# mcahny/vps

Hardware: AMD Instinct MI355X
Metric: frames/sec FuseTrack 1024x2048 (higher is better)
Workload: dtype f32-grade: f16x3 split operands (fp16 pair with scaled residual, 22 significand bits) on MFMA, f32 accumulate

## Files before the change

### include/vps_hip.h

```cpp
#ifndef VPS_HIP_H
#define VPS_HIP_H

#include <stdint.h>

#ifdef __cplusplus
extern "C" {
#endif

int vps_abi_version(void);
const char* vps_build_info(void);

enum { VPS_ACT_NONE = 0, VPS_ACT_RELU = 1, VPS_ACT_LEAKY = 2 };
enum { VPS_PREC_F32 = 0, VPS_PREC_BF16 = 1, VPS_PREC_BF16X3 = 2, VPS_PREC_BF16X6 = 3, VPS_PREC_F16X3 = 4 };

typedef struct vps_conv_desc {
    const float* in;
    int32_t N, H, W;
    int32_t in_ld;
    int32_t in_coff;
    int32_t cin_pad;
    const float* w;
    int32_t cout, cout_pad, kpad;
    int32_t KH, KW, stride;
    int32_t pad_y[2], pad_x[2];
// ... 13 lines not shown
    int32_t off_ld;
    int32_t tile_n;
    int32_t ksplit;
    float* ws;
    int32_t prec;
    const void* w_split;
    int32_t korder;
    int32_t* status;
    double* gn_stats;
    int32_t gn_cpg, gn_rep;
    int32_t* tile_counter;
    const void* w_thin;
} vps_conv_desc;

int vps_conv2d(const vps_conv_desc* d, void* stream);

typedef struct vps_tensor4 {
    float* p;
    int64_t sn, sc, sh, sw;
} vps_tensor4;

int vps_resample2d(vps_tensor4 in, vps_tensor4 flow, vps_tensor4 out,
                   int B, int C, int H, int W, void* stream);

int vps_channelnorm(vps_tensor4 in, vps_tensor4 out, int B, int C, int H, int W, void* stream);

int vps_correlation(const float* in1, int ld1, int coff1, const float* in2, int ld2, int coff2,
                    float* out, int out_ld, int out_coff,
                    int N, int H, int W, int C, int max_disp, int stride2,
                    int act, float slope, void* stream);
// ... 1 lines not shown
                        float* out, int out_ld, int out_coff, int N, int H, int W, int C,
                        int max_disp, int stride2, int act, float slope, int32_t* status, void* stream);

int vps_flow_warp(const float* in, int in_ld, int in_coff, const float* flow, int flow_ld, int flow_coff,
                  float* out, int out_ld, int out_coff, int N, int H, int W, int C, void* stream);

int vps_nchw_to_nhwc(const float* in, float* out, int out_ld, int out_coff, int N, int C, int H, int W,
                     int Cpad, void* stream);
int vps_nhwc_to_nchw(const float* in, int in_ld, int in_coff, float* out, int N, int C, int H, int W, void* stream);

int vps_resize(const float* in, int in_ld, int in_coff, int Hi, int Wi,
               float* out, int out_ld, int out_coff, int Ho, int Wo,
               int N, int C, int mode, float alpha, void* stream);
int vps_pool3x3s2(const float* in, int in_ld, int in_coff, int Hi, int Wi,
                  float* out, int out_ld, int out_coff, int N, int C, int mode, void* stream);
int vps_bfp_gather(const float* const* levels, const int* ld, const int* ratio, int nlevels,
                   float* out, int out_ld, int out_coff, int N, int H0, int W0, int C, void* stream);
int vps_bfp_scatter(const float* bsf, int bsf_ld, const float* level, int lvl_ld, float* out, int out_ld,
                    int N, int H0, int W0, int C, int ratio, void* stream);
int vps_bfp_scatter_all(const float* bsf, int bsf_ld, const float* const* levels, const int* lvl_ld, float* const* outs,
                        const int* out_ld, int nlevels, int N, int H0, int W0, int C, void* stream);
int vps_axpb(const float* in, int in_ld, int in_coff, float* out, int out_ld, int out_coff,
             int64_t npix, int C, float a, float b, void* stream);

int vps_flow_prep(const float* img, const float* ref, const float* mean3, const float* std3,
                  float* out, int out_ld, int H, int W, double* partial, int nblk, float* rgb_mean_out,
                  void* stream);
int vps_flow_prep_pad(const float* img, const float* ref, const float* mean3, const float* std3,
                      float* out, int out_ld, int H, int W, int Hp, int Wp, double* partial, int nblk, float* rgb_mean_out,
                      void* stream);
// ... 4 lines not shown

int vps_flow_stage_full(const float* x6, int x_ld, const float* flow_a, int a_ld, int a_coff,
                        const float* flow_b, int b_ld, int b_coff, int H, int W, int mode, float mul,
                        float* out, int out_ld, void* stream);

int vps_groupnorm_relu(const float* in, int in_ld, float* out, int out_ld, int out_coff, int64_t npix, int C, int G,
                       const float* gamma, const float* beta, float eps, int relu,
                       double* stats, void* stream);
int vps_groupnorm_apply(const float* in, int in_ld, float* out, int out_ld, int out_coff, int64_t npix, int C, int G,
                        const float* gamma, const float* beta, float eps, int relu,
                        const double* stats, int nrep, void* stream);

int vps_tcea_temporal(const float* emb, int emb_ld, const float* emb_ref, int ref_ld,
                      const float* fea0, int f0_ld, const float* fea1, int f1_ld,
                      float* out, int out_ld, int64_t npix, int C, void* stream);
int vps_tcea_modulate(const float* fea, const float* att, const float* att_add, float* out,
                      int64_t n, void* stream);
int vps_tcea_modulate_ld(const float* fea, int fea_ld, const float* att, int att_ld, const float* att_add, int add_ld,
                         float* out, int out_ld, int64_t npix, int C, void* stream);

int vps_roi_align(const float* const* feats, const int* ld, const int* Hs, const int* Ws, const float* scales,
                  int nlevels, float finest_scale, const float* rois, int R, int C, int P, int sample_num,
                  float* out, void* stream);

int vps_nms_batched(const float* boxes, int nbatch, int nmax, const int32_t* counts_dev, float thr,
                    uint64_t* mask_ws, int32_t* keep, int32_t* nkeep, void* stream);

int vps_delta2bbox(const float* anchors, const float* deltas, const float* scores, float* boxes5, int n,
                   float std_x, float std_y, float std_w, float std_h, float img_h, float img_w, void* stream);

// ... 125 lines not shown
```

### vps_amd/csrc/conv_mfma.hip

```cpp
#include "conv_common.h"

namespace {
template <int TM, int TN, int WAVES_M, int WAVES_N, bool DEFORM>
__global__ __launch_bounds__(256, 2)
void conv_mfma_f32_kernel(const vps_conv_desc d, const int M, const int tiles_m, const int tiles_n,
                          const int ksteps_per_split) {
    constexpr int BN = WAVES_N * TN * 32;
    static_assert(WAVES_M * TM * 32 == BM, "block M tile must be 128");
    static_assert(WAVES_M * WAVES_N == 4, "4 wavefronts per block");
    constexpr int NB = BN / 32;

    __shared__ __attribute__((aligned(16))) float As[BM * LDS_LD];
    __shared__ __attribute__((aligned(16))) float Bs[BN * LDS_LD];

    const int t = threadIdx.x;
    int swz = xcd_swizzle(blockIdx.x, gridDim.x);
    int tile_n, tile_m, cls, split;
    decode_tile(d, swz, tiles_n, tiles_m, tile_n, tile_m, cls, split);

    const int py = cls / d.os_x, px = cls - py * d.os_x;
    const int pad_y = d.pad_y[py], pad_x = d.pad_x[px];
    const float* __restrict__ wcls = d.w + (size_t)cls * d.cout_pad * d.kpad;

    const int H = d.H, W = d.W, KH = d.KH, KW = d.KW, cin_pad = d.cin_pad;
// ... 777 lines not shown
        case CONV_K_H8: vpsi_launch_conv_h8(d, p, s); break;
        case CONV_K_PW: vpsi_launch_conv_pw(d, p, s); break;
        case CONV_K_Q: vpsi_launch_conv_q(d, p, s); break;
        default:
            if (d.tile_n == 128) launch_conv<2, 2, 2, 2>(d, p, s);
            else if (d.tile_n == 64) launch_conv<2, 1, 2, 2>(d, p, s);
            else launch_conv<1, 1, 4, 1>(d, p, s);
    }
    int st = vps_launch_status();
    if (st || !p.needs_reduce) return st;
    const size_t total = (size_t)d.nclass * p.M * d.cout;
    if (p.reduce_v4) hipLaunchKernelGGL(conv_splitk_reduce_kernel<4>, dim3(stream_grid((long)(total / 4), 256)), dim3(256), 0, s, d, p.M);
    else hipLaunchKernelGGL(conv_splitk_reduce_kernel<1>, dim3(stream_grid((long)total, 256)), dim3(256), 0, s, d, p.M);
    return vps_launch_status();
}
```

### vps_amd/csrc/conv_plan.h

```cpp
#pragma once
#include <stddef.h>
#include "../../include/vps_hip.h"

#ifndef VPS_EARG
#define VPS_EARG(x) (-1000 - (x))
#endif

enum conv_kernel {
    CONV_K_NONE = 0,
    CONV_K_SMALL3X3V,
    CONV_K_SMALL_BATCHED,
    CONV_K_SMALL,
    CONV_K_THIN,
    CONV_K_DCN256,
    CONV_K_N16T,
    CONV_K_N32,
    CONV_K_N16,
    CONV_K_H8S2,
    CONV_K_H8P,
    CONV_K_H8,
    CONV_K_HALO,
    CONV_K_PW,
    CONV_K_Q,
    CONV_K_F32,
// ... 29 lines not shown
    bool h8p;
    bool n16t;
    bool n32;
    bool s2_halo;
    bool thin;
    bool debug_occ;
};

struct conv_thin_shape { int c4, ks, s, ph; };
extern const conv_thin_shape conv_thin_shapes[4];

int vpsi_conv_check(const vps_conv_desc& d);
conv_plan vpsi_conv_plan(const vps_conv_desc& d, const conv_limits& lim, const conv_switches& sw);
const char* vpsi_conv_kernel_name(int kernel);

#ifdef __HIPCC__
void vpsi_launch_conv_small(const vps_conv_desc& d, const conv_plan& p, hipStream_t s);
void vpsi_launch_conv_thin(const vps_conv_desc& d, const conv_plan& p, hipStream_t s);
void vpsi_launch_conv_n16(const vps_conv_desc& d, const conv_plan& p, hipStream_t s);
void vpsi_launch_conv_h8(const vps_conv_desc& d, const conv_plan& p, hipStream_t s);
void vpsi_launch_conv_h8p(const vps_conv_desc& d, const conv_plan& p, hipStream_t s);
void vpsi_launch_conv_h8s2(const vps_conv_desc& d, const conv_plan& p, hipStream_t s);
void vpsi_launch_conv_pw(const vps_conv_desc& d, const conv_plan& p, hipStream_t s);
void vpsi_launch_conv_q(const vps_conv_desc& d, const conv_plan& p, hipStream_t s);
void vpsi_conv_pw_limits(conv_limits& lim, bool debug);
void vpsi_conv_thin_limits(conv_limits& lim, bool debug);
void vpsi_conv_q_debug_occ();
#endif
```

### vps_amd/csrc/conv_pw.hip

```cpp
#include "conv_common.h"
#include <cstdio>

namespace {

constexpr int PMODE = VPS_PREC_F16X3;

template <int TN, bool HAS_RES, int NKU>
__global__ __launch_bounds__(256, 2)
void conv_pw_kernel(const vps_conv_desc d, const int M, const int tiles_m, const int tiles_n, const int nk, const int nit) {
    constexpr int TM = 2, WAVES_N = 2;
    constexpr int BN = WAVES_N * TN * 32;
    typedef Split<PMODE> SM;
    typedef _Float16 elem_t;
    typedef vec8<elem_t> x8;
    typedef vec4<elem_t> x4;
    constexpr int NSA = SM::NSA, NSB = SM::NSB, NLB = SM::NLB, NT = SM::NT;
    static_assert(NSA == 2 && NLB == 2 && NSB == 3 && NT == 3, "f16x3");
    constexpr int ABUF = NSA * BM * LDS_LDH;
    constexpr int NFRAG = NLB * 2 * (BN / 32);
    constexpr int BBUF = NFRAG * 512;
    static_assert((NFRAG * 64) % 256 == 0, "whole 16-byte chunks per thread");
    constexpr int NBL = NFRAG * 64 / 256;
    constexpr int NST = TM * TN * 4;

// ... 12 lines not shown

    const int k4 = t & 7;
    const int r0 = t >> 3;
    const int nbt = d.cout_pad >> 5, kst = d.kpad >> 4;
    const size_t wplane = (size_t)nbt * kst * 512;
    const __amdgpu_buffer_rsrc_t wrsrc = make_rsrc(d.w_split, (unsigned)(wplane * NSB * sizeof(elem_t)));
    const unsigned wbase = (unsigned)((((size_t)(tile_n * (BN / 32)) * kst) * 512) * sizeof(elem_t));
    const unsigned wlane = (unsigned)lane * 16u;
    const __amdgpu_buffer_rsrc_t arsrc = make_rsrc(d.in, (unsigned)((size_t)d.N * d.H * d.W * d.in_ld * sizeof(float)));
    const __amdgpu_buffer_rsrc_t orsrc = make_rsrc(d.out, (unsigned)((size_t)d.N * d.Ho * d.Wo * d.out_ld * sizeof(float)));
    const int rs = d.res_shift;
    const __amdgpu_buffer_rsrc_t rrsrc = make_rsrc(HAS_RES ? d.res : d.in, HAS_RES ? (unsigned)((size_t)d.N * (d.Ho >> rs) * (d.Wo >> rs) * d.res_ld * sizeof(float)) : 0u);
    const unsigned ld4 = (unsigned)d.in_ld * 4u;
    const unsigned acoff = (unsigned)(d.in_coff + k4 * 4) * 4u;
    const bool plain = d.stride == 1;

    int lk = 0, lit = 0, bk = 0;
    unsigned rowoff[4];
    auto set_rows = [&](const int it) {
        const int tm = (it * mper + mlocal) * 8 + xcd;
#pragma unroll
        for (int i = 0; i < 4; ++i) {
            const int m = tm * BM + r0 + 32 * i;
            const bool ok = tm < tiles_m && m < M;
            unsigned pix = (unsigned)m;
            if (!plain) {
                const int mm = ok ? m : 0;
                const int qx = mm % d.Qw, tq = mm / d.Qw;
                const int qy = tq % d.Qh, n = tq / d.Qh;
                pix = (unsigned)((n * d.H + qy * d.stride) * d.W + qx * d.stride);
            }
            rowoff[i] = ok ? pix * ld4 + acoff : 0xFFFFFFF0u;
        }
    };
    f32x4 areg[2][4];
    x8 breg[2][NBL];
    float amax = 0.f;

    auto load_A = [&](const int slot) {
        const unsigned koff = (unsigned)lk * (BK * 4u);
#pragma unroll
        for (int i = 0; i < 4; ++i)
            areg[slot][i] = buffer_load16<f32x4>(arsrc, rowoff[i] != 0xFFFFFFF0u ? rowoff[i] + koff : 0xFFFFFFF0u, 0u);
        if (++lk == nk) {
            lk = 0;
            ++lit;
            set_rows(lit);
        }
    };
    auto load_B = [&](const int slot) {
#pragma unroll
        for (int j = 0; j < NBL; ++j) {
            const int f = wave + 4 * j, bcol = f % (BN / 32), pm = f / (BN / 32);
            breg[slot][j] = buffer_load16<x8>(wrsrc, wlane, wbase + (unsigned)(((size_t)(pm >> 1) * wplane + ((size_t)bcol * kst + 2 * bk + (pm & 1)) * 512) * sizeof(elem_t)));
        }
        if (++bk == nk) bk = 0;
    };
    auto store_A = [&](const int i, const int buf, const int slot) {
        x4 sp[NSA];
        split_act<PMODE>(areg[slot][i], sp, amax);
        const int row = r0 + 32 * i;
#pragma unroll
        for (int p = 0; p < NSA; ++p)
            *reinterpret_cast<x4*>(&As[buf * ABUF + p * (BM * LDS_LDH) + row * LDS_LDH + (((k4 >> 1) ^ lds_swz(row)) << 3) + ((k4 & 1) << 2)]) = sp[p];
    };
    auto store_B = [&](const int j, const int buf, const int slot) {
        *reinterpret_cast<x8*>(&Bs[buf * BBUF + (t + 256 * j) * 8]) = breg[slot][j];
    };

    const int frag_row = (wm * TM * 32 + (lane & 31)) * LDS_LDH;
    const int frag_sw = lds_swz(lane & 31);
    const int frag_chunk[2] = {(((lane >> 5)) ^ frag_sw) << 3, ((2 + (lane >> 5)) ^ frag_sw) << 3};
    x8 af[2][NSA][TM];
    x8 bf[NSB][TN];
    auto read_A = [&](const int m, const int buf) {
// ... 222 lines not shown
                for (int a = 0; a < TM; ++a)
#pragma unroll
                    for (int b = 0; b < TN; ++b)
#pragma unroll
                        for (int r = 0; r < 16; ++r) acc[a][b][r] = 0.f;
            }
        }
    }
    report_range<PMODE>(d, amax);
}

}

__attribute__((visibility("hidden")))
void vpsi_conv_pw_limits(conv_limits& lim, bool debug) {
    (void)hipOccupancyMaxActiveBlocksPerMultiprocessor(&lim.pw_per_cu[0], conv_pw_kernel<1, false, 0>, 256, 0);
    (void)hipOccupancyMaxActiveBlocksPerMultiprocessor(&lim.pw_per_cu[1], conv_pw_kernel<2, false, 0>, 256, 0);
    if (debug) for (int tn = 1; tn <= 2; ++tn) fprintf(stderr, "[vps] pointwise kernel <TN %d>: %d blocks/CU\n", tn, lim.pw_per_cu[tn - 1]);
}

__attribute__((visibility("hidden")))
void vpsi_launch_conv_pw(const vps_conv_desc& d, const conv_plan& p, hipStream_t s) {
    const int tn = d.tile_n == 128 ? 2 : 1;
#define VPS_PW_LAUNCH(TNV, RESV, NKV) hipLaunchKernelGGL((conv_pw_kernel<TNV, RESV, NKV>), dim3(p.grid), dim3(p.block), 0, s, d, p.M, p.tiles_m, p.tiles_n, p.nk, p.nit)
#define VPS_PW_NK(TNV, RESV)                                         \
    do {                                                             \
        if (p.nk == 2) VPS_PW_LAUNCH(TNV, RESV, 2);                  \
        else if (p.nk == 4) VPS_PW_LAUNCH(TNV, RESV, 4);             \
        else if (p.nk == 8) VPS_PW_LAUNCH(TNV, RESV, 8);             \
        else VPS_PW_LAUNCH(TNV, RESV, 0);                            \
    } while (0)
    if (d.res) { if (tn == 2) VPS_PW_NK(2, true); else VPS_PW_NK(1, true); }
    else { if (tn == 2) VPS_PW_NK(2, false); else VPS_PW_NK(1, false); }
#undef VPS_PW_NK
#undef VPS_PW_LAUNCH
}
```

### vps_amd/csrc/nn_ops.hip

```cpp
#include "common.h"

typedef float f32x4 __attribute__((ext_vector_type(4)));

namespace {

template <int V> struct vecn { typedef float type; };
template <> struct vecn<4> { typedef f32x4 type; };

template <int V>
__global__ __launch_bounds__(256)
void resize_kernel(const float* __restrict__ in, int in_ld, int in_coff, int Hi, int Wi,
                   float* __restrict__ out, int out_ld, int out_coff, int Ho, int Wo,
                   int N, int C, int mode, float alpha, float sh, float sw) {
    typedef typename vecn<V>::type vt;
    const int cv = C / V;
    const long total = (long)N * Ho * Wo * cv;
    for (long idx = (long)blockIdx.x * blockDim.x + threadIdx.x; idx < total; idx += (long)gridDim.x * blockDim.x) {
        const int c = (int)(idx % cv) * V;
        const int pix = (int)(idx / cv);
        const int x = pix % Wo;
        const int yy = pix / Wo;
        const int y = yy % Ho, n = yy / Ho;
        const float* ib = in + (size_t)n * Hi * Wi * in_ld + in_coff + c;
        vt v;
// ... 43 lines not shown
        }
        vt m = t[4], s = vt{}, zero = vt{};
#pragma unroll
        for (int k = 0; k < 9; ++k) {
            if constexpr (V == 1) { m = fmaxf(m, t[k]); }
            else {
#pragma unroll
                for (int e = 0; e < 4; ++e) m[e] = fmaxf(m[e], t[k][e]);
            }
            s += ok[k] ? t[k] : zero;
        }
        *reinterpret_cast<vt*>(out + (size_t)pix * out_ld + out_coff + c) = mode == 0 ? m : s / 9.0f;
    }
}

struct GatherArgs {
    const float* lv[5];
    int ld[5];
    int ratio[5];
    int n;
};

__global__ __launch_bounds__(256)
void bfp_gather_kernel(GatherArgs a, float* __restrict__ out, int out_ld, int out_coff, int N, int H0, int W0, int C) {
    const int c4n = C >> 2;
    const long total = (long)N * H0 * W0 * c4n;
    const float div = (float)a.n;
    for (long idx = (long)blockIdx.x * blockDim.x + threadIdx.x; idx < total; idx += (long)gridDim.x * blockDim.x) {
        const int c4 = (int)(idx % c4n);
        const long pix = idx / c4n;
// ... 256 lines not shown
            cor0 += __shfl_xor(cor0, off, 64);
            cor1 += __shfl_xor(cor1, off, 64);
        }
        const float p0 = 1.f / (1.f + expf(-cor0));
        const float p1 = 1.f / (1.f + expf(-cor1));
        for (int c4 = lane; c4 < c4n; c4 += 64) {
            const f32x4 f0 = *reinterpret_cast<const f32x4*>(fea0 + (size_t)pix * f0_ld + 4 * c4);
            const f32x4 f1 = *reinterpret_cast<const f32x4*>(fea1 + (size_t)pix * f1_ld + 4 * c4);
            *reinterpret_cast<f32x4*>(out + (size_t)pix * out_ld + 4 * c4) = f0 * p0;
            *reinterpret_cast<f32x4*>(out + (size_t)pix * out_ld + C + 4 * c4) = f1 * p1;
        }
    }
}

__global__ __launch_bounds__(256)
void tcea_modulate_kernel(const float* __restrict__ fea, const float* __restrict__ att, const float* __restrict__ att_add,
                          float* __restrict__ out, long n) {
    for (long i = (long)blockIdx.x * blockDim.x + threadIdx.x; i < n; i += (long)gridDim.x * blockDim.x) {
        const float s = 1.f / (1.f + expf(-att[i]));
        out[i] = fea[i] * s * 2.f + att_add[i];
    }
}

__global__ __launch_bounds__(256)
void tcea_modulate_ld_kernel(const float* __restrict__ fea, int fea_ld, const float* __restrict__ att, int att_ld,
                             const float* __restrict__ att_add, int add_ld, float* __restrict__ out, int out_ld, long npix, int C) {
    const int c4n = C >> 2;
    const long total = npix * c4n;
    for (long i = (long)blockIdx.x * blockDim.x + threadIdx.x; i < total; i += (long)gridDim.x * blockDim.x) {
        const long pix = i / c4n;
// ... 26 lines not shown
                           in, in_ld, in_coff, Hi, Wi, out, out_ld, out_coff, Ho, Wo, N, C, mode, alpha, sh, sw);
    return vps_launch_status();
}

extern "C" int vps_pool3x3s2(const float* in, int in_ld, int in_coff, int Hi, int Wi, float* out, int out_ld, int out_coff,
                             int N, int C, int mode, void* stream) {
    if (!in || !out || N <= 0 || C <= 0 || Hi <= 0 || Wi <= 0) return VPS_EARG(1);
    const int Ho = (Hi + 2 - 3) / 2 + 1, Wo = (Wi + 2 - 3) / 2 + 1;
    if ((long)N * Ho * Wo > 0x7fffffffL) return VPS_EARG(2);
    if (!((C | in_ld | in_coff | out_ld | out_coff) & 3))
        hipLaunchKernelGGL(pool3x3s2_kernel<4>, dim3(stream_grid((long)N * Ho * Wo * (C >> 2), 256)), dim3(256), 0, (hipStream_t)stream,
                           in, in_ld, in_coff, Hi, Wi, out, out_ld, out_coff, Ho, Wo, N, C, mode);
    else
        hipLaunchKernelGGL(pool3x3s2_kernel<1>, dim3(stream_grid((long)N * Ho * Wo * C, 256)), dim3(256), 0, (hipStream_t)stream,
                           in, in_ld, in_coff, Hi, Wi, out, out_ld, out_coff, Ho, Wo, N, C, mode);
    return vps_launch_status();
}

extern "C" int vps_bfp_gather(const float* const* levels, const int* ld, const int* ratio, int nlevels,
                              float* out, int out_ld, int out_coff, int N, int H0, int W0, int C, void* stream) {
    if (!levels || !ld || !ratio || !out || nlevels < 1 || nlevels > 5 || (C & 3) || (out_ld & 3) || (out_coff & 3)) return VPS_EARG(1);
    GatherArgs a;
    a.n = nlevels;
    for (int l = 0; l < 5; ++l) {
        a.lv[l] = l < nlevels ? levels[l] : nullptr;
        a.ld[l] = l < nlevels ? ld[l] : 0;
        a.ratio[l] = l < nlevels ? ratio[l] : 1;
        if (l < nlevels && (!levels[l] || (ld[l] & 3) || ratio[l] < 1 || H0 % ratio[l] || W0 % ratio[l])) return VPS_EARG(2);
    }
    hipLaunchKernelGGL(bfp_gather_kernel, dim3(stream_grid((long)N * H0 * W0 * (C >> 2), 256)), dim3(256), 0,
// ... 78 lines not shown
    return vps_launch_status();
}

extern "C" int vps_tcea_temporal(const float* emb, int emb_ld, const float* emb_ref, int ref_ld,
                                 const float* fea0, int f0_ld, const float* fea1, int f1_ld,
                                 float* out, int out_ld, int64_t npix, int C, void* stream) {
    if (!emb || !emb_ref || !fea0 || !fea1 || !out || npix <= 0 || C <= 0 || (C & 3)) return VPS_EARG(1);
    if ((emb_ld & 3) || (ref_ld & 3) || (f0_ld & 3) || (f1_ld & 3) || (out_ld & 3)) return VPS_EARG(2);
    if (((uintptr_t)emb | (uintptr_t)emb_ref | (uintptr_t)fea0 | (uintptr_t)fea1 | (uintptr_t)out) & 15) return VPS_EARG(3);
    long g = (npix + 3) / 4; if (g > 16384) g = 16384;
    hipLaunchKernelGGL(tcea_temporal_kernel, dim3((unsigned)g), dim3(256), 0, (hipStream_t)stream, emb, emb_ld, emb_ref, ref_ld,
                       fea0, f0_ld, fea1, f1_ld, out, out_ld, (long)npix, C);
    return vps_launch_status();
}

extern "C" int vps_tcea_modulate_ld(const float* fea, int fea_ld, const float* att, int att_ld, const float* att_add, int add_ld,
                                    float* out, int out_ld, int64_t npix, int C, void* stream) {
    if (!fea || !att || !att_add || !out || npix <= 0 || C <= 0) return VPS_EARG(1);
    if ((C | fea_ld | att_ld | add_ld | out_ld) & 3 || (((uintptr_t)fea | (uintptr_t)att | (uintptr_t)att_add | (uintptr_t)out) & 15)) return VPS_EARG(2);
    hipLaunchKernelGGL(tcea_modulate_ld_kernel, dim3(stream_grid((long)npix * (C >> 2), 256)), dim3(256), 0, (hipStream_t)stream, fea, fea_ld,
                       att, att_ld, att_add, add_ld, out, out_ld, (long)npix, C);
    return vps_launch_status();
}

extern "C" int vps_tcea_modulate(const float* fea, const float* att, const float* att_add, float* out, int64_t n, void* stream) {
    if (!fea || !att || !att_add || !out || n <= 0) return VPS_EARG(1);
    hipLaunchKernelGGL(tcea_modulate_kernel, dim3(stream_grid((long)n, 256)), dim3(256), 0, (hipStream_t)stream, fea, att,
                       att_add, out, (long)n);
    return vps_launch_status();
}
// ... 1 lines not shown
```

### vps_amd/hip.py

```python
import ctypes
import os
from ctypes import (POINTER, Structure, byref, c_char_p, c_double, c_float, c_int, c_int32, c_int64, c_uint64,
                    c_void_p)

import torch

_HERE = os.path.dirname(os.path.abspath(__file__))
LIB_PATH = os.environ.get('VPS_HIP_LIB') or os.path.join(_HERE, 'csrc', 'libvpship.so')
ABI_VERSION = 21

ACT_NONE, ACT_RELU, ACT_LEAKY = 0, 1, 2
PREC_F32, PREC_BF16, PREC_BF16X3, PREC_BF16X6, PREC_F16X3 = 0, 1, 2, 3, 4

SYMBOLS = [
    'vps_abi_version', 'vps_build_info', 'vps_conv2d', 'vps_resample2d', 'vps_channelnorm', 'vps_correlation',
    'vps_flow_warp', 'vps_nchw_to_nhwc', 'vps_nhwc_to_nchw', 'vps_resize', 'vps_pool3x3s2', 'vps_bfp_gather',
    'vps_bfp_scatter', 'vps_bfp_scatter_all', 'vps_axpb', 'vps_flow_prep', 'vps_flow_prep_pad', 'vps_flow_stage', 'vps_flow_stage_full', 'vps_groupnorm_relu', 'vps_groupnorm_apply', 'vps_tcea_temporal',
    'vps_tcea_modulate', 'vps_tcea_modulate_ld', 'vps_correlation_f16', 'vps_roi_align', 'vps_nms_batched', 'vps_delta2bbox', 'vps_bbox_overlaps',
    'vps_row_softmax', 'vps_mask_count', 'vps_mask_commit', 'vps_mask_removal', 'vps_mask_removal_dep', 'vps_mask_removal_hist', 'vps_frame_tail', 'vps_mask_level', 'vps_panoptic_combine',
    'vps_panoptic_combine_dev', 'vps_rpn_select', 'vps_rpn_collect', 'vps_maskroi_select', 'vps_maskroi_finish', 'vps_track_assign', 'vps_pan_instances',
    'vps_unify_hist', 'vps_unify_tables', 'vps_unify_write', 'vps_image_prep', 'vps_resize_u8', 'vps_segment_stats', 'vps_segment_paint', 'vps_pair_count',
    'vps_png_info', 'vps_png_decode_bgr8', 'vps_jpeg_info', 'vps_jpeg_decode_coef', 'vps_jpeg_reconstruct',
    'vps_png_encode_bound', 'vps_png_deflate',
    'vps_png_inflate', 'vps_png_reconstruct_ws', 'vps_png_reconstruct', 'vps_png_reconstruct_block_rows',
    'vps_unify_tables_image', 'vps_segment_stats_ch', 'vps_segment_paint_ch', 'vps_sseg_confusion',
    'vps_overlay_render', 'vps_jpeg_quant_tables', 'vps_jpeg_encode_bound', 'vps_jpeg_encode_coef', 'vps_jpeg_write_bound', 'vps_jpeg_write',
    'vps_flow_max_radius', 'vps_flow_colour',
]


class ConvDesc(Structure):
    _fields_ = [
        ('inp', c_void_p), ('N', c_int32), ('H', c_int32), ('W', c_int32),
        ('in_ld', c_int32), ('in_coff', c_int32), ('cin_pad', c_int32),
        ('w', c_void_p), ('cout', c_int32), ('cout_pad', c_int32), ('kpad', c_int32),
        ('KH', c_int32), ('KW', c_int32), ('stride', c_int32),
        ('pad_y', c_int32 * 2), ('pad_x', c_int32 * 2),
        ('out', c_void_p), ('Ho', c_int32), ('Wo', c_int32), ('out_ld', c_int32), ('out_coff', c_int32),
        ('Qh', c_int32), ('Qw', c_int32), ('os_y', c_int32), ('os_x', c_int32), ('nclass', c_int32),
        ('scale', c_void_p), ('shift', c_void_p), ('res', c_void_p),
        ('res_ld', c_int32), ('res_coff', c_int32), ('res_shift', c_int32),
        ('act', c_int32), ('slope', c_float),
        ('offset', c_void_p), ('off_ld', c_int32),
# ... 48 lines not shown
        return _lib
    if not os.path.exists(LIB_PATH):
        raise VpsHipError('libvpship.so not found at %s — build it with `python -c "import __graft_entry__ as g; '
                          'g.build()"` or `make -C vps_amd/csrc`. There is no CPU fallback.' % LIB_PATH)
    lib = ctypes.PyDLL(LIB_PATH)
    missing = [s for s in SYMBOLS if not hasattr(lib, s)]
    if missing:
        raise VpsHipError('libvpship.so is missing symbols: %s' % missing)
    lib.vps_abi_version.restype = c_int
    lib.vps_build_info.restype = c_char_p
    if lib.vps_abi_version() != ABI_VERSION:
        raise VpsHipError('libvpship.so ABI %d != binding ABI %d' % (lib.vps_abi_version(), ABI_VERSION))
    for s in SYMBOLS[2:]:
        getattr(lib, s).restype = c_int
    lib.vps_conv2d.argtypes = [POINTER(ConvDesc), c_void_p]
    lib.vps_resample2d.argtypes = [Tensor4, Tensor4, Tensor4, c_int, c_int, c_int, c_int, c_void_p]
    lib.vps_channelnorm.argtypes = [Tensor4, Tensor4, c_int, c_int, c_int, c_int, c_void_p]
    lib.vps_correlation.argtypes = [c_void_p, c_int, c_int, c_void_p, c_int, c_int, c_void_p, c_int, c_int,
                                    c_int, c_int, c_int, c_int, c_int, c_int, c_int, c_float, c_void_p]
    lib.vps_correlation_f16.argtypes = [c_void_p, c_int, c_int, c_void_p, c_int, c_int, c_void_p, c_int, c_int,
                                        c_int, c_int, c_int, c_int, c_int, c_int, c_int, c_float, c_void_p, c_void_p]
    lib.vps_flow_warp.argtypes = [c_void_p, c_int, c_int, c_void_p, c_int, c_int, c_void_p, c_int, c_int,
                                  c_int, c_int, c_int, c_int, c_void_p]
    lib.vps_nchw_to_nhwc.argtypes = [c_void_p, c_void_p, c_int, c_int, c_int, c_int, c_int, c_int, c_int, c_void_p]
    lib.vps_nhwc_to_nchw.argtypes = [c_void_p, c_int, c_int, c_void_p, c_int, c_int, c_int, c_int, c_void_p]
    lib.vps_resize.argtypes = [c_void_p, c_int, c_int, c_int, c_int, c_void_p, c_int, c_int, c_int, c_int,
                               c_int, c_int, c_int, c_float, c_void_p]
    lib.vps_pool3x3s2.argtypes = [c_void_p, c_int, c_int, c_int, c_int, c_void_p, c_int, c_int, c_int, c_int, c_int,
                                  c_void_p]
    lib.vps_bfp_gather.argtypes = [POINTER(c_void_p), POINTER(c_int), POINTER(c_int), c_int, c_void_p, c_int, c_int,
# ... 138 lines not shown
```

### vps_amd/necks.py

```python
import os

import torch
import torch.nn as nn

from . import hip, nhwc
from .base import HipModule
from .registry import EXTRA_NECKS, NECKS

SCATTER_ALL = os.environ.get('VPS_SCATTER_ALL', '1') != '0'


class _ConvModule(nn.Module):

    def __init__(self, cin, cout, k, padding=0):
        super().__init__()
        self.conv = nn.Conv2d(cin, cout, k, padding=padding)


@NECKS.register_module
class FPN(HipModule):
    def __init__(self, in_channels, out_channels, num_outs, start_level=0, end_level=-1, add_extra_convs=False,
                 **unused):
        super().__init__()
        assert start_level == 0 and end_level == -1 and not add_extra_convs, 'only the fusetrack.py FPN is on the path'
# ... 100 lines not shown
        nhwc.correlation(bsf, warp1, cat.window(C, 81), 4, 1, prec=self._refine.prec)
        x = cat
        for i, pc in enumerate(self._est):
            y = pc(x, ws=ws, name='%sest%d' % (tag, i), temp=True)
            if x is not cat:
                ws.release(x)
            x = y
        flow_fine = x
        warp2 = nhwc.flow_warp(warp1, flow_fine, T('warp2', C))
        ws.release(warp1)
        P = self._t
        emb = T('emb', 2 * C)
        P['tAtt_1'](bsf, out=emb.window(0, C), ws=ws)
        P['tAtt_1'](warp2, out=emb.window(C, C), ws=ws)
        emb_ref = P['tAtt_2'](bsf, ws=ws, name=tag + 'emb_ref', temp=True)
        al = nhwc.tcea_temporal(emb, emb_ref, bsf, warp2, T('aligned', 2 * C))
        ws.release(emb, emb_ref)
        fa = P['fea_att1'](al, ws=ws, name=tag + 'fea_att1', temp=True)
        fea, att = fa.window(0, C), fa.window(C, C)
        ws.release(al)
        Hh, Wh = (H + 1) // 2, (W + 1) // 2
        pooled = ws.fmap(tag + 'attpool', N, Hh, Wh, 2 * C, temp=True)
        nhwc.pool3x3s2(att, pooled.window(0, C), 'max')
        nhwc.pool3x3s2(att, pooled.window(C, C), 'avg')
        att = P['sAtt_2'](pooled, ws=ws, name=tag + 'att2', temp=True)
        ws.release(pooled)
        att3 = P['sAtt_3'](att, ws=ws, name=tag + 'att3', temp=True)
        ws.release(att)
        att_up = nhwc.resize(att3, ws.fmap(tag + 'attup', N, 2 * Hh, 2 * Wh, C, temp=True), 'bilinear')
        ws.release(att3)
        att = P['sAtt_4'](att_up, ws=ws, name=tag + 'att4', temp=True)
        ws.release(att_up)
        add1 = P['sAtt_add_1'](att, ws=ws, name=tag + 'add1', temp=True)
        add = P['sAtt_add_2'](add1, ws=ws, name=tag + 'add2', temp=True)
        ws.release(add1)
        fused = nhwc.tcea_modulate(fea, att, add, T('fused', C))
        ws.release(fa, att, add)
        refined = self._refine(fused, ws=ws, name=tag + 'refined', temp=True)
        outs = [ws.fmap('%sout%d' % (tag, i), lv.N, lv.H, lv.W, C) for i, lv in enumerate(levels)]
# ... 19 lines not shown
```

### vps_amd/nhwc.py

```python
import collections
import ctypes
import os
import weakref
from ctypes import c_float, c_int, c_void_p

import torch

from . import hip


def _ceil(a, b):
    return (a + b - 1) // b * b


_PREC_NAMES = {'f32': hip.PREC_F32, 'bf16': hip.PREC_BF16, 'bf16x3': hip.PREC_BF16X3, 'bf16x6': hip.PREC_BF16X6, 'f16x3': hip.PREC_F16X3}
PREC_NAMES = _PREC_NAMES
_PLANES = {hip.PREC_BF16: 1, hip.PREC_BF16X3: 2, hip.PREC_BF16X6: 3, hip.PREC_F16X3: 3}
MFMA_PRODUCTS = {hip.PREC_F32: 1, hip.PREC_BF16: 1, hip.PREC_BF16X3: 3, hip.PREC_BF16X6: 6, hip.PREC_F16X3: 3}
F16_SLOTS = 4096
_F16_STATUS = {}
_F16_LAYERS = {}
_F16_NEXT = [1]
F16_FALLBACKS = [0]

# ... 417 lines not shown
            d = hit.desc
            self.gn_fused = bool(d.gn_stats)
            hip.conv2d(d)
            return out
        Qh, Qw = (x.H, x.W) if self.transposed else (Ho, Wo)
        geo = conv_geometry(self, x.N, Qh, Qw, out.ld, out.coff, res is not None, None if gn is None else gn[1])
        d = self._describe(x, out, Qh, Qw, res, res_shift, offset, act, gn, geo)
        scratch = self._scratch(d, geo, ws, x.t.device)
        self.gn_fused = geo.gn_cpg > 0
        self._launch(d, x, res is not None)
        if len(self._launches) >= 16:
            self._launches.clear()
        self._launches[key] = _Launch(d, (scratch, x.t, out.t, None if res is None else res.t, None if offset is None else offset.t))
        return out

    def _describe(self, x, out, Qh, Qw, res, res_shift, offset, act, gn, geo):
        d = hip.ConvDesc()
        d.inp = x.t.data_ptr(); d.N, d.H, d.W = x.N, x.H, x.W
        d.in_ld, d.in_coff, d.cin_pad = x.ld, x.coff, self.cin_pad
        d.prec, d.korder = self.prec, self.korder
        if self.prec == hip.PREC_F32:
            d.w = self.w.data_ptr()
        else:
            d.w_split = self.w_split.data_ptr()
            if self.w_thin is not None:
                d.w_thin = self.w_thin.data_ptr()
        if self.prec == hip.PREC_F16X3:
            d.status = f16_status(x.t.device).data_ptr() + 4 * self.f16_slot
        d.cout, d.cout_pad, d.kpad = self.cout, self.cout_pad, self.kpad
        d.KH, d.KW, d.stride = self.KH, self.KW, self.stride
# ... 71 lines not shown

def pack_linear(weight, bias, act=hip.ACT_NONE, device='cuda', chw=None, prec=None):
    w = weight.detach().float().cpu()
    if chw is not None:
        C, S = chw
        w = w.view(w.shape[0], C, S).permute(0, 2, 1).reshape(w.shape[0], C * S)
    return PackedConv(w.view(w.shape[0], w.shape[1], 1, 1), bias, None, 1, 0, act=act, device=device, prec=prec)


def resize(x, out, mode='bilinear', alpha=1.0):
    hip.check(hip.load().vps_resize(x.ptr(), x.ld, x.coff, x.H, x.W, out.ptr(), out.ld, out.coff, out.H, out.W,
                                    x.N, x.C, 0 if mode == 'bilinear' else 1, float(alpha), hip.stream_ptr()), 'vps_resize')
    return out


def pool3x3s2(x, out, mode='max'):
    hip.check(hip.load().vps_pool3x3s2(x.ptr(), x.ld, x.coff, x.H, x.W, out.ptr(), out.ld, out.coff, x.N, x.C,
                                       0 if mode == 'max' else 1, hip.stream_ptr()), 'vps_pool3x3s2')
    return out


CORR_F16 = [os.environ.get('VPS_CORR_F16', '1') != '0']
F16_CORR_SLOT = F16_SLOTS - 1


def correlation(x1, x2, out, max_disp, stride2, act=hip.ACT_NONE, slope=0.1, prec=None):
    assert x1.C == x2.C
    if prec == hip.PREC_F16X3 and CORR_F16[0]:
        st = c_void_p(f16_status(x1.t.device).data_ptr() + 4 * F16_CORR_SLOT)
        hip.check(hip.load().vps_correlation_f16(x1.ptr(), x1.ld, x1.coff, x2.ptr(), x2.ld, x2.coff, out.ptr(), out.ld, out.coff,
# ... 69 lines not shown
                                       hip.ptr(out), hip.stream_ptr()), 'vps_roi_align')
    return out


def tcea_temporal(emb, emb_ref, fea0, fea1, out):
    C = fea0.C
    assert emb.C == 2 * C and emb.coff == 0 and emb_ref.coff == 0 and out.coff == 0 and out.C == 2 * C
    assert fea0.coff % 4 == 0 and fea1.coff % 4 == 0
    p0 = c_void_p(fea0.t.data_ptr() + 4 * fea0.coff)
    p1 = c_void_p(fea1.t.data_ptr() + 4 * fea1.coff)
    hip.check(hip.load().vps_tcea_temporal(emb.ptr(), emb.ld, emb_ref.ptr(), emb_ref.ld, p0, fea0.ld, p1, fea1.ld,
                                           out.ptr(), out.ld, out.npix, C, hip.stream_ptr()), 'vps_tcea_temporal')
    return out


def tcea_modulate(fea, att, att_add, out):
    if all(m.coff == 0 and m.C == m.ld for m in (fea, att, att_add, out)):
        hip.check(hip.load().vps_tcea_modulate(fea.ptr(), att.ptr(), att_add.ptr(), out.ptr(), out.t.numel(), hip.stream_ptr()),
                  'vps_tcea_modulate')
        return out
    w = lambda m: c_void_p(m.t.data_ptr() + 4 * m.coff)
    assert fea.C == att.C == att_add.C == out.C and all(m.coff % 4 == 0 for m in (fea, att, att_add, out))
    hip.check(hip.load().vps_tcea_modulate_ld(w(fea), fea.ld, w(att), att.ld, w(att_add), att_add.ld, w(out), out.ld, out.npix, out.C,
                                              hip.stream_ptr()), 'vps_tcea_modulate_ld')
    return out
```

Measured before the change: 56.25.

## Fuse TCEA temporal scaling into pointwise conv loader and merge max/avg pooling

The aligned tensor used to be materialized by tcea_temporal and then read by the fea_att1 pointwise conv. Now a small kernel computes only per-pixel sigmoid correlation probabilities, and the pointwise conv reads bsf and warp2 directly from two sources, scaling each A row by its probability inside the loader. This removes a full write and re-read of the 2C-channel aligned tensor. Separately, the max and avg 3x3 stride-2 pools now run as one kernel that reads the input once. The cost is extra per-row probability loads and resource-descriptor selection inside the conv A loader, plus a fallback path when the planner does not pick the pointwise kernel.

```diff
diff --git a/include/vps_hip.h b/include/vps_hip.h
--- a/include/vps_hip.h
+++ b/include/vps_hip.h
@@ -51,6 +51,8 @@
 } vps_conv_desc;
 
 int vps_conv2d(const vps_conv_desc* d, void* stream);
+int vps_conv_plan_kernel(const vps_conv_desc* d);
+int vps_conv2d_scaled2(const vps_conv_desc* d, const float* in1, int in1_ld, int in1_coff, const float* probs, int dry, void* stream);
 
 typedef struct vps_tensor4 {
     float* p;
@@ -82,6 +84,8 @@
                int N, int C, int mode, float alpha, void* stream);
 int vps_pool3x3s2(const float* in, int in_ld, int in_coff, int Hi, int Wi,
                   float* out, int out_ld, int out_coff, int N, int C, int mode, void* stream);
+int vps_pool3x3s2_maxavg(const float* in, int in_ld, int in_coff, int Hi, int Wi,
+                         float* out, int out_ld, int max_coff, int avg_coff, int N, int C, void* stream);
 int vps_bfp_gather(const float* const* levels, const int* ld, const int* ratio, int nlevels,
                    float* out, int out_ld, int out_coff, int N, int H0, int W0, int C, void* stream);
 int vps_bfp_scatter(const float* bsf, int bsf_ld, const float* level, int lvl_ld, float* out, int out_ld,
@@ -116,6 +120,7 @@
 int vps_tcea_temporal(const float* emb, int emb_ld, const float* emb_ref, int ref_ld,
                       const float* fea0, int f0_ld, const float* fea1, int f1_ld,
                       float* out, int out_ld, int64_t npix, int C, void* stream);
+int vps_tcea_probs(const float* emb, int emb_ld, const float* emb_ref, int ref_ld, float* probs, int64_t npix, int C, void* stream);
 int vps_tcea_modulate(const float* fea, const float* att, const float* att_add, float* out,
                       int64_t n, void* stream);
 int vps_tcea_modulate_ld(const float* fea, int fea_ld, const float* att, int att_ld, const float* att_add, int add_ld,
diff --git a/vps_amd/csrc/conv_mfma.hip b/vps_amd/csrc/conv_mfma.hip
--- a/vps_amd/csrc/conv_mfma.hip
+++ b/vps_amd/csrc/conv_mfma.hip
@@ -815,3 +815,33 @@
     else hipLaunchKernelGGL(conv_splitk_reduce_kernel<1>, dim3(stream_grid((long)total, 256)), dim3(256), 0, s, d, p.M);
     return vps_launch_status();
 }
+
+extern "C" int vps_conv_plan_kernel(const vps_conv_desc* dp) {
+    if (!dp) return VPS_EARG(1);
+    if (const int e = vpsi_conv_check(*dp)) return e;
+    const conv_switches sw = conv_switches_now(*dp);
+    const conv_plan p = vpsi_conv_plan(*dp, conv_limits_once(sw.debug_occ), sw);
+    return p.kernel == CONV_K_NONE ? p.err : p.kernel;
+}
+
+extern "C" int vps_conv2d_scaled2(const vps_conv_desc* dp, const float* in1, int in1_ld, int in1_coff, const float* probs, int dry, void* stream) {
+    if (!dp || !in1 || !probs) return VPS_EARG(1);
+    vps_conv_desc v = *dp;
+    v.in_ld = dp->cin_pad; v.in_coff = 0;
+    if (const int e = vpsi_conv_check(v)) return e;
+    const vps_conv_desc& d = *dp;
+    const int C = d.cin_pad >> 1;
+    if ((d.in_ld & 3) || (d.in_coff & 3) || (in1_ld & 3) || (in1_coff & 3) || d.in_coff < 0 || in1_coff < 0 || d.in_coff + C > d.in_ld || in1_coff + C > in1_ld) return VPS_EARG(30);
+    if (((uintptr_t)in1 & 15) || ((uintptr_t)probs & 7)) return VPS_EARG(31);
+    const conv_switches sw = conv_switches_now(v);
+    const conv_plan p = vpsi_conv_plan(v, conv_limits_once(sw.debug_occ), sw);
+    if (p.kernel == CONV_K_NONE) return p.err;
+    const size_t npix = (size_t)d.N * d.H * d.W;
+    if (p.kernel != CONV_K_PW || (C & 31) || d.stride != 1 || d.res || npix * d.in_ld * sizeof(float) >= 0xFFFFFE00ull ||
+        npix * in1_ld * sizeof(float) >= 0xFFFFFE00ull) return 0;
+    if (dry) return 1;
+    const conv_pw_src2 x2 = {in1, in1_ld, in1_coff, probs};
+    vpsi_launch_conv_pw_scaled2(d, p, x2, (hipStream_t)stream);
+    const int st = vps_launch_status();
+    return st ? st : 1;
+}
diff --git a/vps_amd/csrc/conv_plan.h b/vps_amd/csrc/conv_plan.h
--- a/vps_amd/csrc/conv_plan.h
+++ b/vps_amd/csrc/conv_plan.h
@@ -67,6 +67,12 @@
 conv_plan vpsi_conv_plan(const vps_conv_desc& d, const conv_limits& lim, const conv_switches& sw);
 const char* vpsi_conv_kernel_name(int kernel);
 
+struct conv_pw_src2 {
+    const float* in1;
+    int ld1, coff1;
+    const float* probs;
+};
+
 #ifdef __HIPCC__
 void vpsi_launch_conv_small(const vps_conv_desc& d, const conv_plan& p, hipStream_t s);
 void vpsi_launch_conv_thin(const vps_conv_desc& d, const conv_plan& p, hipStream_t s);
@@ -76,6 +82,7 @@
 void vpsi_launch_conv_h8s2(const vps_conv_desc& d, const conv_plan& p, hipStream_t s);
 void vpsi_launch_conv_pw(const vps_conv_desc& d, const conv_plan& p, hipStream_t s);
 void vpsi_launch_conv_q(const vps_conv_desc& d, const conv_plan& p, hipStream_t s);
+void vpsi_launch_conv_pw_scaled2(const vps_conv_desc& d, const conv_plan& p, const conv_pw_src2& x2, hipStream_t s);
 void vpsi_conv_pw_limits(conv_limits& lim, bool debug);
 void vpsi_conv_thin_limits(conv_limits& lim, bool debug);
 void vpsi_conv_q_debug_occ();
diff --git a/vps_amd/csrc/conv_pw.hip b/vps_amd/csrc/conv_pw.hip
--- a/vps_amd/csrc/conv_pw.hip
+++ b/vps_amd/csrc/conv_pw.hip
@@ -5,9 +5,10 @@
 
 constexpr int PMODE = VPS_PREC_F16X3;
 
-template <int TN, bool HAS_RES, int NKU>
+template <int TN, bool HAS_RES, int NKU, bool SC2 = false>
 __global__ __launch_bounds__(256, 2)
-void conv_pw_kernel(const vps_conv_desc d, const int M, const int tiles_m, const int tiles_n, const int nk, const int nit) {
+void conv_pw_kernel(const vps_conv_desc d, const int M, const int tiles_m, const int tiles_n, const int nk, const int nit, const conv_pw_src2 x2) {
+    static_assert(!SC2 || (NKU == 0 && !HAS_RES), "the scaled two-source loader has instances of the general loop only");
     constexpr int TM = 2, WAVES_N = 2;
     constexpr int BN = WAVES_N * TN * 32;
     typedef Split<PMODE> SM;
@@ -50,6 +51,10 @@
     const unsigned ld4 = (unsigned)d.in_ld * 4u;
     const unsigned acoff = (unsigned)(d.in_coff + k4 * 4) * 4u;
     const bool plain = d.stride == 1;
+    const int nk0 = nk >> 1;
+    const unsigned sz0 = (unsigned)((size_t)d.N * d.H * d.W * d.in_ld * sizeof(float));
+    const unsigned sz1 = SC2 ? (unsigned)((size_t)d.N * d.H * d.W * x2.ld1 * sizeof(float)) : 0u;
+    const __amdgpu_buffer_rsrc_t prsrc = make_rsrc(SC2 ? (const void*)x2.probs : (const void*)d.in, SC2 ? (unsigned)((size_t)M * 2 * sizeof(float)) : 0u);
 
     int lk = 0, lit = 0, bk = 0;
     unsigned rowoff[4];
@@ -66,18 +71,34 @@
                 const int qy = tq % d.Qh, n = tq / d.Qh;
                 pix = (unsigned)((n * d.H + qy * d.stride) * d.W + qx * d.stride);
             }
-            rowoff[i] = ok ? pix * ld4 + acoff : 0xFFFFFFF0u;
+            if constexpr (SC2) rowoff[i] = ok ? pix : 0xFFFFFFF0u;
+            else rowoff[i] = ok ? pix * ld4 + acoff : 0xFFFFFFF0u;
         }
     };
     f32x4 areg[2][4];
+    float preg[2][SC2 ? 4 : 1];
     x8 breg[2][NBL];
     float amax = 0.f;
 
     auto load_A = [&](const int slot) {
-        const unsigned koff = (unsigned)lk * (BK * 4u);
-#pragma unroll
-        for (int i = 0; i < 4; ++i)
-            areg[slot][i] = buffer_load16<f32x4>(arsrc, rowoff[i] != 0xFFFFFFF0u ? rowoff[i] + koff : 0xFFFFFFF0u, 0u);
+        if constexpr (SC2) {
+            const bool h1 = lk >= nk0;
+            const __amdgpu_buffer_rsrc_t srsrc = make_rsrc(h1 ? (const void*)x2.in1 : (const void*)d.in, h1 ? sz1 : sz0);
+            const unsigned sld4 = (unsigned)(h1 ? x2.ld1 : d.in_ld) * 4u;
+            const unsigned soff = (unsigned)((h1 ? x2.coff1 : d.in_coff) + k4 * 4 + (h1 ? lk - nk0 : lk) * BK) * 4u;
+            const unsigned poff = h1 ? 4u : 0u;
+#pragma unroll
+            for (int i = 0; i < 4; ++i) {
+                const bool ok = rowoff[i] != 0xFFFFFFF0u;
+                areg[slot][i] = buffer_load16<f32x4>(srsrc, ok ? rowoff[i] * sld4 + soff : 0xFFFFFFF0u, 0u);
+                preg[slot][i] = __builtin_bit_cast(float, __builtin_amdgcn_raw_buffer_load_b32(prsrc, (int)(ok ? rowoff[i] * 8u + poff : 0xFFFFFFF0u), 0, 0));
+            }
+        } else {
+            const unsigned koff = (unsigned)lk * (BK * 4u);
+#pragma unroll
+            for (int i = 0; i < 4; ++i)
+                areg[slot][i] = buffer_load16<f32x4>(arsrc, rowoff[i] != 0xFFFFFFF0u ? rowoff[i] + koff : 0xFFFFFFF0u, 0u);
+        }
         if (++lk == nk) {
             lk = 0;
             ++lit;
@@ -94,7 +115,9 @@
     };
     auto store_A = [&](const int i, const int buf, const int slot) {
         x4 sp[NSA];
-        split_act<PMODE>(areg[slot][i], sp, amax);
+        f32x4 v = areg[slot][i];
+        if constexpr (SC2) v = v * preg[slot][i];
+        split_act<PMODE>(v, sp, amax);
         const int row = r0 + 32 * i;
 #pragma unroll
         for (int p = 0; p < NSA; ++p)
@@ -347,15 +370,16 @@
 
 __attribute__((visibility("hidden")))
 void vpsi_conv_pw_limits(conv_limits& lim, bool debug) {
-    (void)hipOccupancyMaxActiveBlocksPerMultiprocessor(&lim.pw_per_cu[0], conv_pw_kernel<1, false, 0>, 256, 0);
-    (void)hipOccupancyMaxActiveBlocksPerMultiprocessor(&lim.pw_per_cu[1], conv_pw_kernel<2, false, 0>, 256, 0);
+    (void)hipOccupancyMaxActiveBlocksPerMultiprocessor(&lim.pw_per_cu[0], conv_pw_kernel<1, false, 0, false>, 256, 0);
+    (void)hipOccupancyMaxActiveBlocksPerMultiprocessor(&lim.pw_per_cu[1], conv_pw_kernel<2, false, 0, false>, 256, 0);
     if (debug) for (int tn = 1; tn <= 2; ++tn) fprintf(stderr, "[vps] pointwise kernel <TN %d>: %d blocks/CU\n", tn, lim.pw_per_cu[tn - 1]);
 }
 
 __attribute__((visibility("hidden")))
 void vpsi_launch_conv_pw(const vps_conv_desc& d, const conv_plan& p, hipStream_t s) {
     const int tn = d.tile_n == 128 ? 2 : 1;
-#define VPS_PW_LAUNCH(TNV, RESV, NKV) hipLaunchKernelGGL((conv_pw_kernel<TNV, RESV, NKV>), dim3(p.grid), dim3(p.block), 0, s, d, p.M, p.tiles_m, p.tiles_n, p.nk, p.nit)
+    const conv_pw_src2 x2 = {};
+#define VPS_PW_LAUNCH(TNV, RESV, NKV) hipLaunchKernelGGL((conv_pw_kernel<TNV, RESV, NKV, false>), dim3(p.grid), dim3(p.block), 0, s, d, p.M, p.tiles_m, p.tiles_n, p.nk, p.nit, x2)
 #define VPS_PW_NK(TNV, RESV)                                         \
     do {                                                             \
         if (p.nk == 2) VPS_PW_LAUNCH(TNV, RESV, 2);                  \
@@ -368,3 +392,9 @@
 #undef VPS_PW_NK
 #undef VPS_PW_LAUNCH
 }
+
+__attribute__((visibility("hidden")))
+void vpsi_launch_conv_pw_scaled2(const vps_conv_desc& d, const conv_plan& p, const conv_pw_src2& x2, hipStream_t s) {
+    if (d.tile_n == 128) hipLaunchKernelGGL((conv_pw_kernel<2, false, 0, true>), dim3(p.grid), dim3(p.block), 0, s, d, p.M, p.tiles_m, p.tiles_n, p.nk, p.nit, x2);
+    else hipLaunchKernelGGL((conv_pw_kernel<1, false, 0, true>), dim3(p.grid), dim3(p.block), 0, s, d, p.M, p.tiles_m, p.tiles_n, p.nk, p.nit, x2);
+}
diff --git a/vps_amd/csrc/nn_ops.hip b/vps_amd/csrc/nn_ops.hip
--- a/vps_amd/csrc/nn_ops.hip
+++ b/vps_amd/csrc/nn_ops.hip
@@ -81,6 +81,44 @@
     }
 }
 
+template <int V>
+__global__ __launch_bounds__(256)
+void pool3x3s2_maxavg_kernel(const float* __restrict__ in, int in_ld, int in_coff, int Hi, int Wi,
+                             float* __restrict__ out, int out_ld, int max_coff, int avg_coff, int Ho, int Wo, int N, int C) {
+    typedef typename vecn<V>::type vt;
+    const int cv = C / V;
+    const long total = (long)N * Ho * Wo * cv;
+    for (long idx = (long)blockIdx.x * blockDim.x + threadIdx.x; idx < total; idx += (long)gridDim.x * blockDim.x) {
+        const int c = (int)(idx % cv) * V;
+        const int pix = (int)(idx / cv);
+        const int x = pix % Wo;
+        const int yy0 = pix / Wo;
+        const int y = yy0 % Ho, n = yy0 / Ho;
+        const float* ib = in + (size_t)n * Hi * Wi * in_ld + in_coff + c;
+        vt t[9];
+        bool ok[9];
+#pragma unroll
+        for (int k = 0; k < 9; ++k) {
+            const int yy = 2 * y + k / 3 - 1, xx = 2 * x + k % 3 - 1;
+            ok[k] = (unsigned)yy < (unsigned)Hi && (unsigned)xx < (unsigned)Wi;
+            const int yc = min(max(yy, 0), Hi - 1), xc = min(max(xx, 0), Wi - 1);
+            t[k] = *reinterpret_cast<const vt*>(ib + ((size_t)yc * Wi + xc) * in_ld);
+        }
+        vt m = t[4], s = vt{}, zero = vt{};
+#pragma unroll
+        for (int k = 0; k < 9; ++k) {
+            if constexpr (V == 1) { m = fmaxf(m, t[k]); }
+            else {
+#pragma unroll
+                for (int e = 0; e < 4; ++e) m[e] = fmaxf(m[e], t[k][e]);
+            }
+            s += ok[k] ? t[k] : zero;
+        }
+        *reinterpret_cast<vt*>(out + (size_t)pix * out_ld + max_coff + c) = m;
+        *reinterpret_cast<vt*>(out + (size_t)pix * out_ld + avg_coff + c) = s / 9.0f;
+    }
+}
+
 struct GatherArgs {
     const float* lv[5];
     int ld[5];
@@ -367,6 +405,33 @@
 }
 
 __global__ __launch_bounds__(256)
+void tcea_probs_kernel(const float* __restrict__ emb, int emb_ld, const float* __restrict__ emb_ref, int ref_ld,
+                       float* __restrict__ probs, long npix, int C) {
+    const int lane = threadIdx.x & 63, wave = threadIdx.x >> 6;
+    const int c4n = C >> 2;
+    for (long pix = (long)blockIdx.x * 4 + wave; pix < npix; pix += (long)gridDim.x * 4) {
+        float cor0 = 0.f, cor1 = 0.f;
+        for (int c4 = lane; c4 < c4n; c4 += 64) {
+            const f32x4 r = *reinterpret_cast<const f32x4*>(emb_ref + (size_t)pix * ref_ld + 4 * c4);
+            const f32x4 e0 = *reinterpret_cast<const f32x4*>(emb + (size_t)pix * emb_ld + 4 * c4);
+            const f32x4 e1 = *reinterpret_cast<const f32x4*>(emb + (size_t)pix * emb_ld + C + 4 * c4);
+            cor0 += e0[0] * r[0] + e0[1] * r[1] + e0[2] * r[2] + e0[3] * r[3];
+            cor1 += e1[0] * r[0] + e1[1] * r[1] + e1[2] * r[2] + e1[3] * r[3];
+        }
+        for (int off = 32; off >= 1; off >>= 1) {
+            cor0 += __shfl_xor(cor0, off, 64);
+            cor1 += __shfl_xor(cor1, off, 64);
+        }
+        const float p0 = 1.f / (1.f + expf(-cor0));
+        const float p1 = 1.f / (1.f + expf(-cor1));
+        if (lane == 0) {
+            probs[2 * pix] = p0;
+            probs[2 * pix + 1] = p1;
+        }
+    }
+}
+
+__global__ __launch_bounds__(256)
 void tcea_modulate_kernel(const float* __restrict__ fea, const float* __restrict__ att, const float* __restrict__ att_add,
                           float* __restrict__ out, long n) {
     for (long i = (long)blockIdx.x * blockDim.x + threadIdx.x; i < n; i += (long)gridDim.x * blockDim.x) {
@@ -423,6 +488,21 @@
     else
         hipLaunchKernelGGL(pool3x3s2_kernel<1>, dim3(stream_grid((long)N * Ho * Wo * C, 256)), dim3(256), 0, (hipStream_t)stream,
                            in, in_ld, in_coff, Hi, Wi, out, out_ld, out_coff, Ho, Wo, N, C, mode);
+    return vps_launch_status();
+}
+
+extern "C" int vps_pool3x3s2_maxavg(const float* in, int in_ld, int in_coff, int Hi, int Wi, float* out, int out_ld, int max_coff, int avg_coff,
+                                    int N, int C, void* stream) {
+    if (!in || !out || N <= 0 || C <= 0 || Hi <= 0 || Wi <= 0) return VPS_EARG(1);
+    const int Ho = (Hi + 2 - 3) / 2 + 1, Wo = (Wi + 2 - 3) / 2 + 1;
+    if ((long)N * Ho * Wo > 0x7fffffffL) return VPS_EARG(2);
+    if (max_coff < 0 || avg_coff < 0 || max_coff + C > out_ld || avg_coff + C > out_ld || (max_coff < avg_coff + C && avg_coff < max_coff + C)) return VPS_EARG(3);
+    if (!((C | in_ld | in_coff | out_ld | max_coff | avg_coff) & 3))
+        hipLaunchKernelGGL(pool3x3s2_maxavg_kernel<4>, dim3(stream_grid((long)N * Ho * Wo * (C >> 2), 256)), dim3(256), 0, (hipStream_t)stream,
+                           in, in_ld, in_coff, Hi, Wi, out, out_ld, max_coff, avg_coff, Ho, Wo, N, C);
+    else
+        hipLaunchKernelGGL(pool3x3s2_maxavg_kernel<1>, dim3(stream_grid((long)N * Ho * Wo * C, 256)), dim3(256), 0, (hipStream_t)stream,
+                           in, in_ld, in_coff, Hi, Wi, out, out_ld, max_coff, avg_coff, Ho, Wo, N, C);
     return vps_launch_status();
 }
 
@@ -531,6 +611,15 @@
     return vps_launch_status();
 }
 
+extern "C" int vps_tcea_probs(const float* emb, int emb_ld, const float* emb_ref, int ref_ld, float* probs, int64_t npix, int C, void* stream) {
+    if (!emb || !emb_ref || !probs || npix <= 0 || C <= 0 || (C & 3)) return VPS_EARG(1);
+    if ((emb_ld & 3) || (ref_ld & 3) || emb_ld < 2 * C || ref_ld < C) return VPS_EARG(2);
+    if ((((uintptr_t)emb | (uintptr_t)emb_ref) & 15) || ((uintptr_t)probs & 7)) return VPS_EARG(3);
+    long g = (npix + 3) / 4; if (g > 16384) g = 16384;
+    hipLaunchKernelGGL(tcea_probs_kernel, dim3((unsigned)g), dim3(256), 0, (hipStream_t)stream, emb, emb_ld, emb_ref, ref_ld, probs, (long)npix, C);
+    return vps_launch_status();
+}
+
 extern "C" int vps_tcea_modulate_ld(const float* fea, int fea_ld, const float* att, int att_ld, const float* att_add, int add_ld,
                                     float* out, int out_ld, int64_t npix, int C, void* stream) {
     if (!fea || !att || !att_add || !out || npix <= 0 || C <= 0) return VPS_EARG(1);
diff --git a/vps_amd/hip.py b/vps_amd/hip.py
--- a/vps_amd/hip.py
+++ b/vps_amd/hip.py
@@ -26,7 +26,9 @@
     'vps_unify_tables_image', 'vps_segment_stats_ch', 'vps_segment_paint_ch', 'vps_sseg_confusion',
     'vps_overlay_render', 'vps_jpeg_quant_tables', 'vps_jpeg_encode_bound', 'vps_jpeg_encode_coef', 'vps_jpeg_write_bound', 'vps_jpeg_write',
     'vps_flow_max_radius', 'vps_flow_colour',
+    'vps_conv_plan_kernel', 'vps_conv2d_scaled2', 'vps_tcea_probs', 'vps_pool3x3s2_maxavg',
 ]
+CONV_K_PW = 13
 
 
 class ConvDesc(Structure):
@@ -105,6 +107,10 @@
     for s in SYMBOLS[2:]:
         getattr(lib, s).restype = c_int
     lib.vps_conv2d.argtypes = [POINTER(ConvDesc), c_void_p]
+    lib.vps_conv_plan_kernel.argtypes = [POINTER(ConvDesc)]
+    lib.vps_conv2d_scaled2.argtypes = [POINTER(ConvDesc), c_void_p, c_int, c_int, c_void_p, c_int, c_void_p]
+    lib.vps_tcea_probs.argtypes = [c_void_p, c_int, c_void_p, c_int, c_void_p, c_int64, c_int, c_void_p]
+    lib.vps_pool3x3s2_maxavg.argtypes = [c_void_p, c_int, c_int, c_int, c_int, c_void_p, c_int, c_int, c_int, c_int, c_int, c_void_p]
     lib.vps_resample2d.argtypes = [Tensor4, Tensor4, Tensor4, c_int, c_int, c_int, c_int, c_void_p]
     lib.vps_channelnorm.argtypes = [Tensor4, Tensor4, c_int, c_int, c_int, c_int, c_void_p]
     lib.vps_correlation.argtypes = [c_void_p, c_int, c_int, c_void_p, c_int, c_int, c_void_p, c_int, c_int,
diff --git a/vps_amd/necks.py b/vps_amd/necks.py
--- a/vps_amd/necks.py
+++ b/vps_amd/necks.py
@@ -8,6 +8,7 @@
 from .registry import EXTRA_NECKS, NECKS
 
 SCATTER_ALL = os.environ.get('VPS_SCATTER_ALL', '1') != '0'
+NECK_FUSED = os.environ.get('VPS_NECK_FUSED', '1') != '0'
 
 
 class _ConvModule(nn.Module):
@@ -138,15 +139,30 @@
         P['tAtt_1'](bsf, out=emb.window(0, C), ws=ws)
         P['tAtt_1'](warp2, out=emb.window(C, C), ws=ws)
         emb_ref = P['tAtt_2'](bsf, ws=ws, name=tag + 'emb_ref', temp=True)
-        al = nhwc.tcea_temporal(emb, emb_ref, bsf, warp2, T('aligned', 2 * C))
-        ws.release(emb, emb_ref)
-        fa = P['fea_att1'](al, ws=ws, name=tag + 'fea_att1', temp=True)
+        fa, pc = None, P['fea_att1']
+        if NECK_FUSED and pc.prec == hip.PREC_F16X3:
+            probs = ws.get(tag + 'tprobs', (N * H * W, 2), zero=False)
+            fa = T('fea_att1', 2 * C)
+            if pc.scaled_pair(bsf, warp2, probs, fa, ws=ws, dry=True):
+                nhwc.tcea_probs(emb, emb_ref, probs)
+                pc.scaled_pair(bsf, warp2, probs, fa, ws=ws)
+                ws.release(emb, emb_ref)
+            else:
+                ws.release(fa)
+                fa = None
+        if fa is None:
+            al = nhwc.tcea_temporal(emb, emb_ref, bsf, warp2, T('aligned', 2 * C))
+            ws.release(emb, emb_ref)
+            fa = pc(al, ws=ws, name=tag + 'fea_att1', temp=True)
+            ws.release(al)
         fea, att = fa.window(0, C), fa.window(C, C)
-        ws.release(al)
         Hh, Wh = (H + 1) // 2, (W + 1) // 2
         pooled = ws.fmap(tag + 'attpool', N, Hh, Wh, 2 * C, temp=True)
-        nhwc.pool3x3s2(att, pooled.window(0, C), 'max')
-        nhwc.pool3x3s2(att, pooled.window(C, C), 'avg')
+        if NECK_FUSED:
+            nhwc.pool3x3s2_maxavg(att, pooled.window(0, C), pooled.window(C, C))
+        else:
+            nhwc.pool3x3s2(att, pooled.window(0, C), 'max')
+            nhwc.pool3x3s2(att, pooled.window(C, C), 'avg')
         att = P['sAtt_2'](pooled, ws=ws, name=tag + 'att2', temp=True)
         ws.release(pooled)
         att3 = P['sAtt_3'](att, ws=ws, name=tag + 'att3', temp=True)
diff --git a/vps_amd/nhwc.py b/vps_amd/nhwc.py
--- a/vps_amd/nhwc.py
+++ b/vps_amd/nhwc.py
@@ -455,6 +455,28 @@
         self._launches[key] = _Launch(d, (scratch, x.t, out.t, None if res is None else res.t, None if offset is None else offset.t))
         return out
 
+    def scaled_pair(self, x0, x1, probs, out, ws=None, dry=False):
+        C = self.cin // 2
+        assert self.KH == self.KW == 1 and not self.transposed and not self.deform and x0.C == x1.C == C and 2 * C == self.cin_pad
+        assert (x0.N, x0.H, x0.W) == (x1.N, x1.H, x1.W) == (out.N, out.H, out.W) and out.C == self.cout and probs.numel() == 2 * x0.npix
+        key = ('scaled_pair', x0.t.data_ptr(), x0.N, x0.H, x0.W, x0.ld, x0.coff, x1.t.data_ptr(), x1.ld, x1.coff, probs.data_ptr(),
+               out.t.data_ptr(), out.ld, out.coff, _stream_key())
+        hit = self._launches.get(key)
+        if hit is None:
+            geo = conv_geometry(self, x0.N, x0.H, x0.W, out.ld, out.coff, False, None)
+            d = self._describe(x0, out, x0.H, x0.W, None, 0, None, None, None, geo)
+            scratch = self._scratch(d, geo, ws, x0.t.device)
+            if len(self._launches) >= 16:
+                self._launches.clear()
+            hit = self._launches[key] = _Launch(d, [scratch, x0.t, x1.t, probs, out.t, None])
+        if dry and hit.keep[-1] is not None:
+            return hit.keep[-1]
+        rc = hip.load().vps_conv2d_scaled2(ctypes.byref(hit.desc), hip.ptr(x1.t), x1.ld, x1.coff, hip.ptr(probs), 1 if dry else 0, hip.stream_ptr())
+        if rc < 0:
+            hip.check(rc, 'vps_conv2d_scaled2')
+        hit.keep[-1] = rc == 1
+        return rc == 1
+
     def _describe(self, x, out, Qh, Qw, res, res_shift, offset, act, gn, geo):
         d = hip.ConvDesc()
         d.inp = x.t.data_ptr(); d.N, d.H, d.W = x.N, x.H, x.W
@@ -556,6 +578,13 @@
     return out
 
 
+def pool3x3s2_maxavg(x, out_max, out_avg):
+    assert out_max.t is out_avg.t and out_max.C == out_avg.C == x.C
+    hip.check(hip.load().vps_pool3x3s2_maxavg(x.ptr(), x.ld, x.coff, x.H, x.W, out_max.ptr(), out_max.ld, out_max.coff, out_avg.coff,
+                                              x.N, x.C, hip.stream_ptr()), 'vps_pool3x3s2_maxavg')
+    return out_max, out_avg
+
+
 def pool3x3s2(x, out, mode='max'):
     hip.check(hip.load().vps_pool3x3s2(x.ptr(), x.ld, x.coff, x.H, x.W, out.ptr(), out.ld, out.coff, x.N, x.C,
                                        0 if mode == 'max' else 1, hip.stream_ptr()), 'vps_pool3x3s2')
@@ -655,6 +684,14 @@
     return out
 
 
+def tcea_probs(emb, emb_ref, probs):
+    C = emb_ref.C
+    assert emb.C == 2 * C and emb.coff % 4 == 0 and emb_ref.coff % 4 == 0 and probs.dtype == torch.float32 and probs.numel() == 2 * emb.npix
+    w = lambda m: c_void_p(m.t.data_ptr() + 4 * m.coff)
+    hip.check(hip.load().vps_tcea_probs(w(emb), emb.ld, w(emb_ref), emb_ref.ld, hip.ptr(probs), emb.npix, C, hip.stream_ptr()), 'vps_tcea_probs')
+    return probs
+
+
 def tcea_modulate(fea, att, att_add, out):
     if all(m.coff == 0 and m.C == m.ld for m in (fea, att, att_add, out)):
         hip.check(hip.load().vps_tcea_modulate(fea.ptr(), att.ptr(), att_add.ptr(), out.ptr(), out.t.numel(), hip.stream_ptr()),
```

Result: no change. 56.52 (median of 6 runs) (+0.5%).
